# ChainBreak/denoising_diffusion_deep_fake

Measured on AMD Instinct MI355X. Metric: training images/sec (256x256 U-Net, bs=16/GPU), higher is better.
Workload: dtype f32; 1 GPU; d3f train_denoiser step: noise blend -> Unet(resnet34) fwd -> (MSE+1-SSIM)/2 -> bwd -> Adam, 256x256 synthetic face crops, bs=16/GPU, random-init weights, train-mode BatchNorm; image_size=256, batch_per_gpu=16, global_batch=16, parallelism=dp1, graph_step=False, adam_overlap_tail=False, adam_overlap_tail_steps=0, ranks_seen=1, csrc_digest=87bcf01c09701563

## Files before the change

denoising_diffusion_deep_fake_amd/csrc/conv_wgrad_patch.hip:

```cpp
#include "common.h"

#include <cstdlib>

namespace d3f {

constexpr int PT_TH = 8;

template <int MT> struct PAcc;
template <> struct PAcc<32> { using T = f32x16; static constexpr int N = 16; };
template <> struct PAcc<16> { using T = f32x4; static constexpr int N = 4; };

template <int MT> __device__ __forceinline__ void pmma(typename PAcc<MT>::T& c, float a, float b);
template <> __device__ __forceinline__ void pmma<32>(f32x16& c, float a, float b) {
  c = __builtin_amdgcn_mfma_f32_32x32x2f32(a, b, c, 0, 0, 0);
}
template <> __device__ __forceinline__ void pmma<16>(f32x4& c, float a, float b) {
  c = __builtin_amdgcn_mfma_f32_16x16x4f32(a, b, c, 0, 0, 0);
}

template <typename T> __device__ __forceinline__ void patch_store_f32(float* dst, const uint4& v);
template <> __device__ __forceinline__ void patch_store_f32<float>(float* dst, const uint4& v) {
  *reinterpret_cast<uint4*>(dst) = v;
}
template <> __device__ __forceinline__ void patch_store_f32<bf16_t>(float* dst, const uint4& v) {
  *reinterpret_cast<uint4*>(dst) = make_uint4(v.x << 16, v.x & 0xffff0000u, v.y << 16, v.y & 0xffff0000u);
  *reinterpret_cast<uint4*>(dst + 4) = make_uint4(v.z << 16, v.z & 0xffff0000u, v.w << 16, v.w & 0xffff0000u);
}

template <typename T, int MT, int CI_T, int KS, int S, int TW, int CR = CI_T>
__global__ __launch_bounds__(256) void conv_wgrad_patch_kernel(const WgradParams pin) {
  const WgradParams p = wgrad_params_of_net(pin, (int)blockIdx.z);
  constexpr int VE = Elem<T>::VE;
  constexpr int CO_T = MT;
  constexpr bool HALFV = CI_T < VE;
  static_assert(!HALFV || (CI_T == 4 && VE == 8), "half vectors: 4 of 8 bf16 channels");
  constexpr int PH = (PT_TH - 1) * S + KS, PW = (TW - 1) * S + KS;
  constexpr int KSTEP = (MT == 32) ? 2 : 4;
  static_assert(CR == CI_T || (CR < CI_T && CI_T < MT), "fewer columns than staged channels: small-channel path only");
  constexpr int NCOL = KS * KS * CR;
  constexpr int NNT = (NCOL + MT - 1) / MT;
  constexpr int LXS = (CI_T >= 32) ? (MT == 16 ? CI_T + 16 : CI_T + 4) : CI_T;
  constexpr int LYS = (MT == 32) ? CO_T + 4 : CO_T;
  constexpr int XF = PH * PW * LXS, YF = PT_TH * TW * LYS;
  constexpr int RED = 4 * MT * MT;
  constexpr int LDS_F = (XF + YF > RED) ? XF + YF : RED;
  __shared__ __attribute__((aligned(16))) float lds[LDS_F];
  float* Xs = lds;
  float* Ys = lds + XF;

  const int tid = threadIdx.x, lane = tid & 63, wave = tid >> 6;
  const int lc = lane & (MT - 1);
  const int lg = lane / MT;
  const int Cin = p.slab_cin;
  const int ci_slices = HALFV ? 1 : Cin / CI_T;
  const int slice = blockIdx.y;
  const int cil0 = (slice % ci_slices) * CI_T;
  const int ci0 = p.ci_base + cil0, co0 = (slice / ci_slices) * CO_T;
  const bool from0 = ci0 < p.C0;
  const int Cs = from0 ? p.C0 : p.C1;
  const int sh = from0 ? p.shift0 : 0;
  const int Hs = from0 ? p.H0s : p.Hv;
  const int Ws = from0 ? p.W0s : p.Wv;
  const int cl0 = from0 ? ci0 : ci0 - p.C0;
  const __amdgpu_buffer_rsrc_t rdy = make_rsrc(p.dy, p.dy_bytes);
  const __amdgpu_buffer_rsrc_t rx = from0 ? make_rsrc(p.src0, p.src0_bytes) : make_rsrc(p.src1, p.src1_bytes);

  int loff[(CI_T >= MT) ? 1 : NNT];
  if (CI_T < MT) {
#pragma unroll
    for (int j = 0; j < NNT; ++j) {
      const int n = j * MT + lc;
      int tap = n / CR;
      const int c = n - tap * CR;
      if (tap >= KS * KS) tap = KS * KS - 1;
      const int kh = tap / KS, kw = tap - kh * KS;
      loff[(CI_T >= MT) ? 0 : j] = (kh * PW + kw) * LXS + c;
    }
  }

  typename PAcc<MT>::T acc[NNT];
#pragma unroll
  for (int j = 0; j < NNT; ++j)
#pragma unroll
    for (int r = 0; r < PAcc<MT>::N; ++r) acc[j][r] = 0.f;

  const int tiles_x = (p.Wo + TW - 1) / TW, tiles_y = (p.Ho + PT_TH - 1) / PT_TH;
  const int ntiles = p.B * tiles_y * tiles_x;
  constexpr int VX = HALFV ? 1 : CI_T / VE, VY = CO_T / VE;

  constexpr int NVX = (PH * PW * VX + 255) / 256, NVY = (PT_TH * TW * VY + 255) / 256;
  uint4 rxv[NVX], ryv[NVY];
  auto issue_loads = [&](int t) {
    const int b = t / (tiles_y * tiles_x);
    const int tr = t - b * tiles_y * tiles_x;
    const int oy0 = (tr / tiles_x) * PT_TH, ox0 = (tr % tiles_x) * TW;
#pragma unroll
    for (int i = 0; i < NVX; ++i) {
      const int v = tid + i * 256;
      const int pix = v / VX, cv = v - pix * VX;
      const int py = pix / PW, px = pix - py * PW;
      const int iy = oy0 * S - p.pad + py, ix = ox0 * S - p.pad + px;
      const bool ok = v < PH * PW * VX && (unsigned)iy < (unsigned)p.Hv && (unsigned)ix < (unsigned)p.Wv;
      const int gp = (b * Hs + (iy >> sh)) * Ws + (ix >> sh);
      rxv[i] = buf_load16(rx, ok ? (unsigned)(gp * Cs + cl0 + cv * VE) * (unsigned)sizeof(T) : BUF_OOB);
    }
#pragma unroll
    for (int i = 0; i < NVY; ++i) {
      const int v = tid + i * 256;
      const int pix = v / VY, cv = v - pix * VY;
      const int y = pix / TW, x = pix - y * TW;
      const int oy = oy0 + y, ox = ox0 + x;
      const int co = co0 + cv * VE;
      const bool ok = v < PT_TH * TW * VY && oy < p.Ho && ox < p.Wo && co < p.Cout;
      ryv[i] = buf_load16(rdy, ok ? (unsigned)(((b * p.Ho + oy) * p.Wo + ox) * p.Cout + co) * (unsigned)sizeof(T) : BUF_OOB);
    }
  };
  auto store_tile = [&]() {
#pragma unroll
    for (int i = 0; i < NVX; ++i) {
      const int v = tid + i * 256;
      const int pix = v / VX, cv = v - pix * VX;
      if (v < PH * PW * VX) {
        if constexpr (HALFV)
          *reinterpret_cast<uint4*>(&Xs[pix * LXS]) =
              make_uint4(rxv[i].x << 16, rxv[i].x & 0xffff0000u, rxv[i].y << 16, rxv[i].y & 0xffff0000u);
        else
          patch_store_f32<T>(&Xs[pix * LXS + cv * VE], rxv[i]);
      }
    }
#pragma unroll
    for (int i = 0; i < NVY; ++i) {
      const int v = tid + i * 256;
      const int pix = v / VY, cv = v - pix * VY;
      if (v < PT_TH * TW * VY) patch_store_f32<T>(&Ys[pix * LYS + cv * VE], ryv[i]);
    }
  };

  if ((int)blockIdx.x < ntiles) issue_loads(blockIdx.x);
  for (int t = blockIdx.x; t < ntiles; t += gridDim.x) {
    __syncthreads();
    store_tile();
    __syncthreads();
    if (t + (int)gridDim.x < ntiles) issue_loads(t + gridDim.x);
#pragma unroll
    for (int yy = 0; yy < PT_TH / 4; ++yy) {
      const int y = wave * (PT_TH / 4) + yy;
      const float* __restrict__ yrow = Ys + (y * TW + lg) * LYS + lc;
      const float* __restrict__ xrow = Xs + ((y * S) * PW + lg * S) * LXS + ((CI_T >= MT) ? lc : 0);
#pragma unroll
      for (int xs = 0; xs < TW / KSTEP; ++xs) {
        const float a = yrow[xs * KSTEP * LYS];
        const float* __restrict__ xb = xrow + xs * KSTEP * S * LXS;
#pragma unroll
        for (int j = 0; j < NNT; ++j) {
          float bv;
          if (CI_T >= MT) {
            constexpr int per_tap = CI_T / MT;
            const int tap = j / per_tap, cb = (j % per_tap) * MT;
            const int kh = tap / KS, kw = tap % KS;
            bv = xb[(kh * PW + kw) * LXS + cb];
          } else {
            bv = xb[loff[(CI_T >= MT) ? 0 : j]];
          }
          pmma<MT>(acc[j], a, bv);
        }
      }
    }
  }

  const int taps = KS * KS;
  float* __restrict__ slab = p.partial + (long)blockIdx.x * p.Cout * taps * Cin;
  float* red = lds;
#pragma unroll
  for (int j = 0; j < NNT; ++j) {
    __syncthreads();
#pragma unroll
    for (int r = 0; r < PAcc<MT>::N; ++r) {
      const int co_l = (MT == 32) ? ((r & 3) + 8 * (r >> 2) + 4 * lg) : (4 * lg + r);
      red[(wave * MT + co_l) * MT + lc] = acc[j][r];
    }
    __syncthreads();
    for (int e = tid; e < MT * MT; e += 256) {
      const float s = (red[e] + red[MT * MT + e]) + (red[2 * MT * MT + e] + red[3 * MT * MT + e]);
      const int co = co0 + e / MT;
      const int n = j * MT + (e % MT);
      const int tap = n / CR, ci = cil0 + (n - tap * CR);
      if (co < p.Cout && tap < taps) {
        slab[((long)co * taps + tap) * Cin + ci] = s;
        if constexpr (HALFV && CR == CI_T) slab[((long)co * taps + tap) * Cin + ci + CI_T] = 0.f;
      }
    }
  }
  if constexpr (CR < CI_T) {
    const int npad = Cin - CR;
    for (int e = tid; e < MT * taps * npad; e += 256) {
      const int c = CR + e % npad, q = e / npad, tap = q % taps, co = co0 + q / taps;
      if (co < p.Cout) slab[((long)co * taps + tap) * Cin + c] = 0.f;
    }
  }
}

template <typename T, int MT, int CI_T, int TW>
__global__ __launch_bounds__(256) void conv_wgrad_patch_cls_kernel(const WgradParams pin) {
  const WgradParams p = wgrad_params_of_net(pin, (int)blockIdx.z);
  constexpr int VE = Elem<T>::VE;
  constexpr int CO_T = MT;
  constexpr int RH = PT_TH / 2;
  static_assert(RH == 4, "one tile row of the parity per wave");
  constexpr int PHL = PT_TH / 2 + 2, PWL = TW / 2 + 2;
  constexpr int KSTEP = (MT == 32) ? 2 : 4;
  constexpr int NCT = CI_T / MT;
  constexpr int NNT = 8 * NCT;
  static_assert(CI_T % MT == 0, "whole column tiles per folded tap");
  constexpr int LXS = (MT == 16 ? CI_T + 16 : CI_T + 4);
  constexpr int LYS = (MT == 32) ? CO_T + 4 : CO_T;
  constexpr int XF = PHL * PWL * LXS, YF = RH * TW * LYS;
  constexpr int RED = 4 * MT * MT;
  constexpr int LDS_F = (XF + YF > RED) ? XF + YF : RED;
  __shared__ __attribute__((aligned(16))) float lds[LDS_F];
  float* Xs = lds;
  float* Ys = lds + XF;

  const int tid = threadIdx.x, lane = tid & 63, wave = tid >> 6;
  const int lc = lane & (MT - 1);
  const int lg = lane / MT;
  const int Cin = p.slab_cin;
  const int ci_slices = Cin / CI_T;
  int slice = blockIdx.y;
  const int py = slice & 1;
  slice >>= 1;
  const int ci0 = (slice % ci_slices) * CI_T, co0 = (slice / ci_slices) * CO_T;
  const __amdgpu_buffer_rsrc_t rdy = make_rsrc(p.dy, p.dy_bytes);
  const __amdgpu_buffer_rsrc_t rx = make_rsrc(p.src0, p.src0_bytes);

  typename PAcc<MT>::T acc[NNT];
#pragma unroll
  for (int j = 0; j < NNT; ++j)
#pragma unroll
    for (int r = 0; r < PAcc<MT>::N; ++r) acc[j][r] = 0.f;

  const int tiles_x = (p.Wo + TW - 1) / TW, tiles_y = (p.Ho + PT_TH - 1) / PT_TH;
  const int ntiles = p.B * tiles_y * tiles_x;
  constexpr int VX = CI_T / VE, VY = CO_T / VE;
  constexpr int NVX = (PHL * PWL * VX + 255) / 256, NVY = (RH * TW * VY + 255) / 256;
  uint4 rxv[NVX], ryv[NVY];
  auto issue_loads = [&](int t) {
    const int b = t / (tiles_y * tiles_x);
    const int tr = t - b * tiles_y * tiles_x;
    const int oy0 = (tr / tiles_x) * PT_TH, ox0 = (tr % tiles_x) * TW;
    const int ly0 = oy0 / 2 - 1, lx0 = ox0 / 2 - 1;
#pragma unroll
    for (int i = 0; i < NVX; ++i) {
      const int v = tid + i * 256;
      const int pix = v / VX, cv = v - pix * VX;
      const int yy = pix / PWL, xx = pix - yy * PWL;
      const int iy = ly0 + yy, ix = lx0 + xx;
      const bool ok = v < PHL * PWL * VX && (unsigned)iy < (unsigned)p.H0s && (unsigned)ix < (unsigned)p.W0s;
      const int gp = (b * p.H0s + iy) * p.W0s + ix;
      rxv[i] = buf_load16(rx, ok ? (unsigned)(gp * p.C0 + ci0 + cv * VE) * (unsigned)sizeof(T) : BUF_OOB);
    }
#pragma unroll
    for (int i = 0; i < NVY; ++i) {
      const int v = tid + i * 256;
      const int pix = v / VY, cv = v - pix * VY;
      const int r = pix / TW, x = pix - r * TW;
      const int oy = oy0 + 2 * r + py, ox = ox0 + x;
      const int co = co0 + cv * VE;
      const bool ok = v < RH * TW * VY && oy < p.Ho && ox < p.Wo && co < p.Cout;
      ryv[i] = buf_load16(rdy, ok ? (unsigned)(((b * p.Ho + oy) * p.Wo + ox) * p.Cout + co) * (unsigned)sizeof(T) : BUF_OOB);
    }
  };
  auto store_tile = [&]() {
#pragma unroll
    for (int i = 0; i < NVX; ++i) {
      const int v = tid + i * 256;
      const int pix = v / VX, cv = v - pix * VX;
      if (v < PHL * PWL * VX) patch_store_f32<T>(&Xs[pix * LXS + cv * VE], rxv[i]);
    }
#pragma unroll
    for (int i = 0; i < NVY; ++i) {
      const int v = tid + i * 256;
      const int pix = v / VY, cv = v - pix * VY;
      if (v < RH * TW * VY) patch_store_f32<T>(&Ys[pix * LYS + cv * VE], ryv[i]);
    }
  };

  if ((int)blockIdx.x < ntiles) issue_loads(blockIdx.x);
  for (int t = blockIdx.x; t < ntiles; t += gridDim.x) {
    __syncthreads();
    store_tile();
    __syncthreads();
    if (t + (int)gridDim.x < ntiles) issue_loads(t + gridDim.x);
    const float* __restrict__ yrow = Ys + (wave * TW) * LYS + lc;
#pragma unroll
    for (int px = 0; px < 2; ++px) {
#pragma unroll
      for (int xs = 0; xs < (TW / 2) / KSTEP; ++xs) {
        const int il = lg + xs * KSTEP;
        const float a = yrow[(2 * il + px) * LYS];
#pragma unroll
        for (int fa = 0; fa < 2; ++fa)
#pragma unroll
          for (int fb = 0; fb < 2; ++fb) {
            const float* __restrict__ xb = Xs + ((wave + fa + py) * PWL + il + fb + px) * LXS + lc;
#pragma unroll
            for (int jc = 0; jc < NCT; ++jc) pmma<MT>(acc[((px * 2 + fa) * 2 + fb) * NCT + jc], a, xb[jc * MT]);
          }
      }
    }
  }

  float* __restrict__ slab = p.partial + (long)blockIdx.x * p.Cout * 16 * Cin;
  float* red = lds;
#pragma unroll
  for (int j = 0; j < NNT; ++j) {
    __syncthreads();
#pragma unroll
    for (int r = 0; r < PAcc<MT>::N; ++r) {
      const int co_l = (MT == 32) ? ((r & 3) + 8 * (r >> 2) + 4 * lg) : (4 * lg + r);
      red[(wave * MT + co_l) * MT + lc] = acc[j][r];
    }
    __syncthreads();
    const int f8 = j / NCT, jc = j - f8 * NCT;
    const int tap = py * 8 + f8;
    for (int e = tid; e < MT * MT; e += 256) {
      const float s = (red[e] + red[MT * MT + e]) + (red[2 * MT * MT + e] + red[3 * MT * MT + e]);
      const int co = co0 + e / MT;
      const int ci = ci0 + jc * MT + (e % MT);
      if (co < p.Cout) slab[((long)co * 16 + tap) * Cin + ci] = s;
    }
  }
}


constexpr int PB_TW = 16;
__global__ __launch_bounds__(256) void conv_wgrad_patch_bf16_kernel(const WgradParams pin) {
  const WgradParams p = wgrad_params_of_net(pin, (int)blockIdx.z);
  typedef short v4s __attribute__((ext_vector_type(4)));
  constexpr int TW = PB_TW, KS = 3, PH = PT_TH + 2, PW = TW + 2;
  constexpr int XB = PH * PW * 64, YB = PT_TH * TW * 64;
  constexpr int RED = 4 * 32 * 32;
  constexpr int LDS_B = (XB + YB > RED * 4) ? XB + YB : RED * 4;
  __shared__ __attribute__((aligned(16))) unsigned char ldsb[LDS_B];
  unsigned char* Xs = ldsb;
  unsigned char* Ys = ldsb + XB;

  const int tid = threadIdx.x, lane = tid & 63, wave = tid >> 6;
  const int Cin = p.slab_cin;
  const int ci_slices = (Cin + 31) / 32;
  const int slice = blockIdx.y;
  const int cil0 = (slice % ci_slices) * 32;
  const int ci0 = p.ci_base + cil0, co0 = (slice / ci_slices) * 32;
  const bool from0 = ci0 < p.C0;
  const int Cs = from0 ? p.C0 : p.C1;
  const int sh = from0 ? p.shift0 : 0;
  const int Hs = from0 ? p.H0s : p.Hv;
  const int Ws = from0 ? p.W0s : p.Wv;
  const int cl0 = from0 ? ci0 : ci0 - p.C0;
  const int xreal = min(32, Cs - cl0), yreal = min(32, p.Cout - co0);
  const __amdgpu_buffer_rsrc_t rdy = make_rsrc(p.dy, p.dy_bytes);
  const __amdgpu_buffer_rsrc_t rx = from0 ? make_rsrc(p.src0, p.src0_bytes) : make_rsrc(p.src1, p.src1_bytes);

  f32x16 acc[KS * KS];
#pragma unroll
  for (int j = 0; j < KS * KS; ++j)
#pragma unroll
    for (int r = 0; r < 16; ++r) acc[j][r] = 0.f;

  const int tiles_x = (p.Wo + TW - 1) / TW, tiles_y = (p.Ho + PT_TH - 1) / PT_TH;
  const int ntiles = p.B * tiles_y * tiles_x;
  constexpr int NVX = (PH * PW * 4 + 255) / 256, NVY = (PT_TH * TW * 4 + 255) / 256;
  uint4 rxv[NVX], ryv[NVY];
  auto issue_loads = [&](int t) {
    const int b = t / (tiles_y * tiles_x);
    const int tr = t - b * tiles_y * tiles_x;
    const int oy0 = (tr / tiles_x) * PT_TH, ox0 = (tr % tiles_x) * TW;
#pragma unroll
    for (int i = 0; i < NVX; ++i) {
      const int v = tid + i * 256;
      const int pix = v >> 2, cv = v & 3;
      const int py = pix / PW, px = pix - py * PW;
      const int iy = oy0 - p.pad + py, ix = ox0 - p.pad + px;
      const bool ok = v < PH * PW * 4 && cv * 8 < xreal && (unsigned)iy < (unsigned)p.Hv && (unsigned)ix < (unsigned)p.Wv;
      const int gp = (b * Hs + (iy >> sh)) * Ws + (ix >> sh);
      rxv[i] = buf_load16(rx, ok ? (unsigned)(gp * Cs + cl0 + cv * 8) * 2u : BUF_OOB);
    }
#pragma unroll
    for (int i = 0; i < NVY; ++i) {
      const int v = tid + i * 256;
      const int pix = v >> 2, cv = v & 3;
      const int y = pix / TW, x = pix - y * TW;
      const int oy = oy0 + y, ox = ox0 + x;
      const bool ok = v < PT_TH * TW * 4 && cv * 8 < yreal && oy < p.Ho && ox < p.Wo;
      ryv[i] = buf_load16(rdy, ok ? (unsigned)(((b * p.Ho + oy) * p.Wo + ox) * p.Cout + co0 + cv * 8) * 2u : BUF_OOB);
    }
  };
  auto store_tile = [&]() {
#pragma unroll
    for (int i = 0; i < NVX; ++i) {
      const int v = tid + i * 256;
      if (v < PH * PW * 4) *reinterpret_cast<uint4*>(Xs + v * 16) = rxv[i];
    }
#pragma unroll
    for (int i = 0; i < NVY; ++i) {
      const int v = tid + i * 256;
      if (v < PT_TH * TW * 4) *reinterpret_cast<uint4*>(Ys + v * 16) = ryv[i];
    }
  };
  const int lg = lane >> 4, q = (lane & 15) >> 2, pq = lane & 3;
  const int rd_lane = ((lg >> 1) * 8 + q) * 64 + ((lg & 1) * 16 + 4 * pq) * 2;
  auto frag = [&](const unsigned char* base) {
    union { uint4 u; v4s h[2]; } f;
#pragma unroll
    for (int h = 0; h < 2; ++h)
      f.h[h] = __builtin_amdgcn_ds_read_tr16_b64_v4i16((__attribute__((address_space(3))) v4s*)(base + rd_lane + h * 4 * 64));
    return f.u;
  };

  if ((int)blockIdx.x < ntiles) issue_loads(blockIdx.x);
  for (int t = blockIdx.x; t < ntiles; t += gridDim.x) {
    __syncthreads();
    store_tile();
    __syncthreads();
    if (t + (int)gridDim.x < ntiles) issue_loads(t + gridDim.x);
#pragma unroll
    for (int yy = 0; yy < PT_TH / 4; ++yy) {
      const int y = wave * (PT_TH / 4) + yy;
      const uint4 a = frag(Ys + (y * TW) * 64);
#pragma unroll
      for (int tap = 0; tap < KS * KS; ++tap) {
        const int kh = tap / KS, kw = tap - kh * KS;
        const uint4 b = frag(Xs + ((y + kh) * PW + kw) * 64);
        acc[tap] = __builtin_amdgcn_mfma_f32_32x32x16_bf16(*reinterpret_cast<const bf16x8*>(&a),
                                                           *reinterpret_cast<const bf16x8*>(&b), acc[tap], 0, 0, 0);
      }
    }
  }

  const int taps = KS * KS;
  float* __restrict__ slab = p.partial + (long)blockIdx.x * p.Cout * taps * Cin;
  float* red = reinterpret_cast<float*>(ldsb);
  const int lc = lane & 31, lh = lane >> 5;
#pragma unroll
  for (int j = 0; j < KS * KS; ++j) {
    __syncthreads();
#pragma unroll
    for (int r = 0; r < 16; ++r) red[(wave * 32 + (r & 3) + 8 * (r >> 2) + 4 * lh) * 32 + lc] = acc[j][r];
    __syncthreads();
    for (int e = tid; e < 32 * 32; e += 256) {
      const float sum = (red[e] + red[1024 + e]) + (red[2048 + e] + red[3072 + e]);
      const int co = co0 + (e >> 5), cil = e & 31;
      if (co < p.Cout && cil < xreal) slab[((long)co * taps + j) * Cin + cil0 + cil] = sum;
    }
  }
}

int wgrad_patch_variant(const WgradParams& p, int dtype) {
  const int cin = p.C0 + p.C1;
  if (p.KH != p.KW) return 0;
  constexpr int maxco = 128;
  constexpr int maxci = 384;
  if (dtype == D3F_BF16 && p.KH == 3 && p.stride == 1 && p.pad == 1 && p.Cout <= maxco && (cin == 16 || (cin % 32 == 0 && cin <= maxci)) &&
      (p.C1 == 0 || p.C0 % 32 == 0) && (p.C0 % 8) == 0 && (p.C1 % 8) == 0 && (p.Cout % 8) == 0)
    return 7;
  if (p.KH == 3 && p.stride == 1 && p.pad == 1) {
    if (p.Cout <= 16 && cin % 32 == 0 && cin <= 64 && (p.C1 == 0 || p.C0 % 32 == 0)) return 1;
    if (p.Cout <= 16 && cin == 16) return 2;
    if (p.Cout == 32 && cin % 32 == 0 && cin <= 128 && (p.C1 == 0 || p.C0 % 32 == 0)) return 3;
  }
  if (dtype == D3F_F32 && p.KH == 7 && p.stride == 2 && p.pad == 3 && cin == 4 && p.C1 == 0 &&
      p.Cout % 32 == 0 && p.Cout <= 64)
    return 4;
  if (dtype == D3F_BF16 && p.KH == 7 && p.stride == 2 && p.pad == 3 && cin == 8 && p.C1 == 0 &&
      p.Cout % 32 == 0 && p.Cout <= 64)
    return (p.cin_real > 0 && p.cin_real <= 4) ? 6 : 5;
  return 0;
}

int wgrad_patch_tiles(const WgradParams& p) { return p.B * cdiv(p.Ho, PT_TH) * cdiv(p.Wo, 16); }

void wgrad_patch_grid(const WgradParams& p, int variant, int* gx, int* gy) {
  const int cin = p.part == WG_WHOLE ? p.C0 + p.C1 : p.part == WG_CLASS ? p.C0 : p.C1;
  const int ci_t = variant == 1 ? 32 : variant == 2 ? 16 : (variant == 3 || variant == 7) ? 32 : (variant == 5 || variant == 6) ? 8 : 4;
  const int co_t = (variant == 3 || variant == 4 || variant == 5 || variant == 6 || variant == 7) ? 32 : 16;
  const int slices = cdiv(cin, ci_t) * cdiv(p.Cout, co_t) * (p.part == WG_CLASS ? 2 : 1);
  const int tiles = wgrad_patch_tiles(p);
  constexpr int g7 = 256;
  static const int gall = prof_knob("D3F_WGRAD_PATCH_WGS") ? atoi(prof_knob("D3F_WGRAD_PATCH_WGS")) : 512;
  int g = (variant == 7 ? g7 : gall) / plan_nets_for(p.plan_nets, 32) / slices;
  if (g > tiles) g = tiles;
  if (g < 1) g = 1;
  *gx = g;
  *gy = slices;
}

template <typename T> static int patch_launch_t(const WgradParams& p, int variant, dim3 grid, hipStream_t stream) {
  const dim3 block(256);
  switch (variant) {
    case 1: hipLaunchKernelGGL((conv_wgrad_patch_kernel<T, 16, 32, 3, 1, 16>), grid, block, 0, stream, p); break;
    case 2: hipLaunchKernelGGL((conv_wgrad_patch_kernel<T, 16, 16, 3, 1, 16>), grid, block, 0, stream, p); break;
    case 3: hipLaunchKernelGGL((conv_wgrad_patch_kernel<T, 32, 32, 3, 1, 16>), grid, block, 0, stream, p); break;
    default: return set_error(-1, "wgrad patch: bad variant %d", variant);
  }
  return 0;
}

int wgrad_patch_launch(const WgradParams& p, int variant, int dtype, hipStream_t stream) {
  int gx, gy;
  wgrad_patch_grid(p, variant, &gx, &gy);
  D3F_CHECK(p.splits == gx, "wgrad patch: params were not planned (splits %d vs %d)", p.splits, gx);
  const dim3 grid((unsigned)gx, (unsigned)gy, (unsigned)nets_of(p.nets)), block(256);
  if (p.cls) {
    D3F_CHECK((variant == 1 || variant == 3) && p.slab_cin == p.C0 && (p.C0 % 32) == 0 && (p.Ho % 2) == 0 && (p.Wo % 2) == 0,
              "wgrad patch: class form needs variant 1 or 3 and whole 32-channel slices of source 0");
    if (dtype == D3F_F32) {
      if (variant == 1) hipLaunchKernelGGL((conv_wgrad_patch_cls_kernel<float, 16, 32, 16>), grid, block, 0, stream, p);
      else hipLaunchKernelGGL((conv_wgrad_patch_cls_kernel<float, 32, 32, 16>), grid, block, 0, stream, p);
    } else {
      if (variant == 1) hipLaunchKernelGGL((conv_wgrad_patch_cls_kernel<bf16_t, 16, 32, 16>), grid, block, 0, stream, p);
      else hipLaunchKernelGGL((conv_wgrad_patch_cls_kernel<bf16_t, 32, 32, 16>), grid, block, 0, stream, p);
    }
    D3F_HIP(hipGetLastError());
    return 0;
  }
  if (variant == 7) {
    D3F_CHECK(dtype == D3F_BF16 && p.part == WG_WHOLE, "wgrad patch: variant 7 is the native bf16 kernel of whole layers");
    hipLaunchKernelGGL(conv_wgrad_patch_bf16_kernel, grid, block, 0, stream, p);
  } else if (variant == 4) {
    D3F_CHECK(dtype == D3F_F32, "wgrad patch: stem variant 4 is the f32 one");
    if (p.cin_real == 3) hipLaunchKernelGGL((conv_wgrad_patch_kernel<float, 32, 4, 7, 2, 16, 3>), grid, block, 0, stream, p);
    else hipLaunchKernelGGL((conv_wgrad_patch_kernel<float, 32, 4, 7, 2, 16>), grid, block, 0, stream, p);
  } else if (variant == 5) {
    D3F_CHECK(dtype == D3F_BF16, "wgrad patch: stem variant 5 is the bf16 one");
    hipLaunchKernelGGL((conv_wgrad_patch_kernel<bf16_t, 32, 8, 7, 2, 16>), grid, block, 0, stream, p);
  } else if (variant == 6) {
    D3F_CHECK(dtype == D3F_BF16, "wgrad patch: stem variant 6 is a bf16 one");
    if (p.cin_real == 3) hipLaunchKernelGGL((conv_wgrad_patch_kernel<bf16_t, 32, 4, 7, 2, 16, 3>), grid, block, 0, stream, p);
    else hipLaunchKernelGGL((conv_wgrad_patch_kernel<bf16_t, 32, 4, 7, 2, 16>), grid, block, 0, stream, p);
  } else if (dtype == D3F_F32) {
    if (int rc = patch_launch_t<float>(p, variant, grid, stream)) return rc;
  } else {
    if (int rc = patch_launch_t<bf16_t>(p, variant, grid, stream)) return rc;
  }
  D3F_HIP(hipGetLastError());
  return 0;
}

}
```

denoising_diffusion_deep_fake_amd/csrc/engine.hip:

```cpp
#include "engine.h"
#include <vector>

#include "head_act.h"

#include <cstdio>
#include <cstdlib>
#include <cstring>

namespace d3f {

constexpr int CS_PP = 16;
__global__ __launch_bounds__(256) void channel_sum_partial_kernel(const float* __restrict__ x, int C, long HW,
                                                                  float* __restrict__ partial, int nb, long net_in,
                                                                  long net_ws) {
  __shared__ float red[256];
  const int seg = blockIdx.x, c = blockIdx.y, b = (int)blockIdx.z % nb;
  if ((int)blockIdx.z >= nb) {
    net_shift(x, net_in); net_shift(partial, net_ws);
  }
  const float* __restrict__ plane = x + ((long)b * C + c) * HW;
  const long per = (HW + CS_PP - 1) / CS_PP, lo = (long)seg * per, hi = lo + per < HW ? lo + per : HW;
  float s = 0.f;
  if ((HW & 3) == 0 && (per & 3) == 0) {
    for (long i = lo + 4 * threadIdx.x; i < hi; i += 4 * 256) {
// ... 644 lines not shown
  frame_.color = mode;
  return 0;
}

int UnetEngine::set_frame_temporal(float strength, int threshold) {
  D3F_CHECK(strength >= 0.f && strength < 1.f, "frame temporal filter: strength %g outside [0, 1) (0 is off)",
            (double)strength);
  D3F_CHECK(threshold >= 1 && threshold <= 255, "frame temporal filter: threshold %d outside 1..255", threshold);
  if (strength == 0.f) strength = 0.f;
  if (memcmp(&strength, &frame_.strength, sizeof(float)) == 0 && threshold == frame_.threshold) return 0;
  if (strength != 0.f) {
    const size_t px = (size_t)H * W;
    D3F_HIP(frame_.state_fake.ensure(px * 3 * sizeof(float)));
    D3F_HIP(frame_.state_real.ensure(px * 3));
    D3F_HIP(frame_.state_coef.ensure(6 * sizeof(float)));
    D3F_HIP(frame_.state_sum.ensure(3 * sizeof(uint64_t)));
    D3F_HIP(frame_.valid.ensure(2 * sizeof(int)));
  }
  drop_frame_graphs();
  frame_.strength = strength;
  frame_.threshold = threshold;
  frame_.reset_pending = true;
  return 0;
}

int UnetEngine::frame_temporal_reset(hipStream_t s) const {
  frame_.reset_pending = false;
  int* valid = frame_.valid.p;
  if (valid == nullptr) return 0;
  if (int rc = temporal_flag_set_launch(valid, 0, s)) return rc;
  return temporal_flag_set_launch(valid + 1, 0, s);
}

void UnetEngine::GraphSlot::destroy() {
  if (exec) (void)hipGraphExecDestroy(exec);
  exec = nullptr;
}

void UnetEngine::drop_frame_graphs() const {
  g_frames_.destroy();
  g_frames_full_.destroy();
}

void UnetEngine::drop_graphs() const {
  g_predict_.destroy();
  g_eval_.destroy();
  drop_frame_graphs();
  if (g_step_) {
    (void)hipGraphExecDestroy(g_step_);
    g_step_ = nullptr;
  }
}

struct Scale255 {
  float mean[3], stdv[3];
  Scale255(const float m[3], const float sd[3]) {
    for (int c = 0; c < 3; ++c) {
      mean[c] = m[c] * 255.0f;
      stdv[c] = sd[c] * 255.0f;
    }
  }
};

int UnetEngine::predict_u8(const float* params_, float* bnstats, const uint8_t* bgr_in, uint8_t* bgr_out,
                           const float mean[3], const float stdv[3], void* ws_, int use_graph,
                           hipStream_t s) const {
  D3F_CHECK(in_channels == 3 && classes == 3, "predict_u8: 3-channel frames only (in %d, out %d)", in_channels, classes);
  char* ws = reinterpret_cast<char*>(ws_);
  const Scale255 k(mean, stdv);
  if (!use_graph) return predict_u8_launches(params_, bnstats, bgr_in, bgr_out, k.mean, k.stdv, ws, s);
  const GraphKey key = {{params_, bnstats, bgr_in, bgr_out, ws_},
                        {k.mean[0], k.mean[1], k.mean[2], k.stdv[0], k.stdv[1], k.stdv[2]}, {}};
  return graph_replay(g_predict_, key, s, [&](hipStream_t gs) {
    return predict_u8_launches(params_, bnstats, bgr_in, bgr_out, k.mean, k.stdv, ws, gs);
  });
}

int UnetEngine::predict_frames(const FrameCall& c, const float* params_, float* bnstats, const float mean[3],
                               const float stdv[3], void* ws_, int use_graph, hipStream_t s) const {
  const bool full = c.full_out != nullptr;
  const char* who = full ? "predict_frames_full_u8" : "predict_frames_u8";
  D3F_CHECK(in_channels == 3 && classes == 3, "%s: 3-channel frames only (in %d, out %d)", who, in_channels, classes);
  char* ws = reinterpret_cast<char*>(ws_);
  const Scale255 k(mean, stdv);
  const FrameOptions& o = frame_;
  const bool aa = o.resample == FRAME_RESAMPLE_CUBIC_AA;
  const bool color = full && o.color == FRAME_COLOR_MEANSTD;
  const bool temporal = o.strength != 0.f;
  uint8_t* const pair = c.pair_out;
  uint8_t* const fake = pair + pair_fake_off();
  const long stride = pair_stride();
  const int32_t* const boxes = c.boxes;
  D3F_CHECK(!(use_graph && boxes),
            "%s with a box per frame cannot be replayed from a graph: a captured launch bakes its kernel arguments in, the "
            "boxes among them, and a graph keyed on their values would be re-captured on every call; pass use_graph = 0",
            who);
  if (int rc = boxes ? (aa ? crop_resize_cubic_aa_boxes_check : crop_resize_cubic_boxes_check)(B, c.src_h, c.src_w, boxes, H,
                                                                                              W, stride)
                     : (aa ? crop_resize_cubic_aa_check : crop_resize_cubic_check)(B, c.src_h, c.src_w, c.x1, c.y1, c.cw,
                                                                                  c.ch, H, W, stride))
    return rc;
  if (full) {
    int rc;
    if (boxes)
      rc = color ? paste_resize_cubic_color_boxes_check(fake, c.raw_in, c.full_out, o.color_coef.p, B, H, W, stride, c.src_h,
                                                        c.src_w, boxes, c.feather)
                 : paste_resize_cubic_boxes_check(fake, c.raw_in, c.full_out, B, H, W, stride, c.src_h, c.src_w, boxes,
                                                  c.feather);
    else
      rc = color ? paste_resize_cubic_color_check(fake, c.raw_in, c.full_out, o.color_coef.p, B, H, W, stride, c.src_h,
                                                  c.src_w, c.x1, c.y1, c.cw, c.ch, c.feather)
                 : paste_resize_cubic_check(fake, c.raw_in, c.full_out, B, H, W, stride, c.src_h, c.src_w, c.x1, c.y1, c.cw,
                                            c.ch, c.feather);
    if (rc) return rc;
    D3F_CHECK(!(use_graph && c.full_out == c.raw_in),
              "predict_frames_full_u8: full_out == raw_in (in place) cannot be replayed from a graph: pass use_graph = 0");
  }
  if (temporal) {
    if (int rc = temporal_filter_check(pair, fake, B, H, W, stride, stride, o.state_fake.p, o.state_real.p, o.valid.p,
                                       o.strength, o.threshold))
      return rc;
    if (o.reset_pending)
      if (int rc = frame_temporal_reset(s)) return rc;
  }
  auto launches = [&](hipStream_t ls) {
    if (int rc = boxes ? (aa ? crop_resize_cubic_aa_boxes_u8_nhwc_launch : crop_resize_cubic_boxes_u8_nhwc_launch)(
                             dtype, c.raw_in, B, c.src_h, c.src_w, boxes, pair, H, W, stride, ws + tensors[t_x].off,
                             tensors[t_x].C, k.mean, k.stdv, ls)
                       : (aa ? crop_resize_cubic_aa_u8_nhwc_launch : crop_resize_cubic_u8_nhwc_launch)(
                             dtype, c.raw_in, B, c.src_h, c.src_w, c.x1, c.y1, c.cw, c.ch, pair, H, W, stride,
                             ws + tensors[t_x].off, tensors[t_x].C, k.mean, k.stdv, ls))
      return rc;
    float* head_out = reinterpret_cast<float*>(ws + head_nchw_off);
    if (int rc = forward_body(params_, bnstats, head_out, ws, 0, ls, nullptr, false)) return rc;
    head_z_live_ = false;
    if (int rc = head_to_u8bgr(ws, fake, stride, k.mean, k.stdv, ls)) return rc;
    if (temporal)
      if (int rc = temporal_filter_u8_launch(pair, fake, B, H, W, stride, stride, o.state_fake.p, o.state_real.p, o.valid.p,
                                             o.strength, o.threshold, ls))
        return rc;
    if (!full) return 0;
    if (!color)
      return boxes ? paste_resize_cubic_boxes_u8_launch(fake, B, H, W, stride, c.raw_in, c.src_h, c.src_w, boxes, c.feather,
                                                        c.full_out, ls)
                   : paste_resize_cubic_u8_launch(fake, B, H, W, stride, c.raw_in, c.src_h, c.src_w, c.x1, c.y1, c.cw, c.ch,
                                                  c.feather, c.full_out, ls);
    int parts = 0;
    if (int rc = channel_sums_pair_slabs_launch(pair, pair_fake_off(), B, H, W, stride, o.color_slabs.p, &parts, ls)) return rc;
    const uint64_t* to = o.color_slabs.p;
    const uint64_t* from = to + (size_t)B * parts * 6;
    if (int rc = color_match_coef_launch(from, to, parts, B, (long)H * W, o.color_coef.p, ls)) return rc;
    if (temporal)
      if (int rc = color_coef_smooth_launch(o.color_coef.p, to, parts, B, (long)H * W, o.strength, o.state_coef.p,
                                            o.state_sum.p, o.valid.p + 1, ls))
        return rc;
    if (boxes)
      return paste_resize_cubic_color_boxes_u8_launch(fake, B, H, W, stride, c.raw_in, c.src_h, c.src_w, boxes, c.feather,
                                                      o.color_coef.p, c.full_out, ls);
    return paste_resize_cubic_color_u8_launch(fake, B, H, W, stride, c.raw_in, c.src_h, c.src_w, c.x1, c.y1, c.cw, c.ch,
                                              c.feather, o.color_coef.p, c.full_out, ls);
  };
  if (!use_graph) return launches(s);
  int strength_bits;
  memcpy(&strength_bits, &o.strength, sizeof(strength_bits));
  const GraphKey key = {{params_, bnstats, c.raw_in, pair, ws_, c.full_out},
                        {k.mean[0], k.mean[1], k.mean[2], k.stdv[0], k.stdv[1], k.stdv[2]},
                        {c.src_h, c.src_w, c.x1, c.y1, c.cw, c.ch, full ? c.feather : 0, full ? o.color : 0, strength_bits,
                         temporal ? o.threshold : 0}};
  return graph_replay(full ? g_frames_full_ : g_frames_, key, s, launches);
}

int UnetEngine::forward_graph(const float* params_, float* bnstats, const float* x, float* out, void* ws_,
                              hipStream_t s) const {
  const GraphKey key = {{params_, bnstats, x, out, ws_}, {}, {}};
  return graph_replay(g_eval_, key, s, [&](hipStream_t gs) { return forward(params_, bnstats, x, out, ws_, 0, gs); });
}

int UnetEngine::train_step_launches(const StepArgs& a, void* ws_, hipStream_t s) const {
  const long per_image = (long)in_channels * H * W;
  if (int rc = pack_weights(a.params, ws_, s)) return rc;
  if (int rc = noise_blend_launch(a.image, a.noise, a.y_uniform, a.lam, a.noisy, nullptr, B, per_image, s)) return rc;
  if (int rc = forward(a.params, a.bnstats, a.noisy, a.pred, ws_, 1, s)) return rc;
  if (int rc = mse_ssim_loss_launch(a.pred, a.image, a.lo, a.hi, a.loss_out, a.gpred, a.loss_ws, B, H, W, s)) return rc;
  if (int rc = backward(a.params, a.gpred, a.grads, ws_, 0, num_segments, s, 1)) return rc;
  return adam_step_dev_launch(a.params, a.grads, a.exp_avg, a.exp_avg_sq, param_floats, a.adam_coef, s);
}

int UnetEngine::train_step(const StepArgs& a, void* ws_, int use_graph, hipStream_t s) const {
  D3F_CHECK(in_channels == 3 && classes == 3, "train_step: the (MSE + 1 - SSIM) / 2 objective is defined on 3-channel images");
  if (!use_graph) return train_step_launches(a, ws_, s);
  if (int rc = wait_for_packed_weights(s)) return rc;
  if (int rc = ensure_streams()) return rc;
  if (gstream_ == nullptr) {
    D3F_HIP(hipStreamCreateWithFlags(&gstream_, hipStreamNonBlocking));
    D3F_HIP(hipEventCreateWithFlags(&ev_gin_, hipEventDisableTiming));
    D3F_HIP(hipEventCreateWithFlags(&ev_gout_, hipEventDisableTiming));
  }
  const bool same = g_step_ != nullptr && g_step_ws_ == ws_ && memcmp(&a, &g_step_key_, sizeof(StepArgs)) == 0;
  if (!same) {
    if (g_step_) {
      (void)hipGraphExecDestroy(g_step_);
      g_step_ = nullptr;
    }
    hipGraph_t graph = nullptr;
    D3F_HIP(hipStreamBeginCapture(gstream_, hipStreamCaptureModeThreadLocal));
    const int rc = train_step_launches(a, ws_, gstream_);
    const hipError_t e = hipStreamEndCapture(gstream_, &graph);
    pack_pending_ = pack_mid_pending_ = false;
    side_dirty_ = false;
    if (rc != 0) {
      if (graph) (void)hipGraphDestroy(graph);
      return rc;
    }
    D3F_HIP(e);
    const hipError_t ei = hipGraphInstantiate(&g_step_, graph, nullptr, nullptr, 0);
    (void)hipGraphDestroy(graph);
    D3F_HIP(ei);
    g_step_key_ = a;
    g_step_ws_ = ws_;
  }
  D3F_HIP(hipGraphLaunch(g_step_, s));
  return 0;
}

int UnetEngine::wait_for_packed_weights(hipStream_t s) const {
  if (pack_mid_pending_) {
    D3F_HIP(hipStreamWaitEvent(s, ev_pack_mid_, 0));
    pack_mid_pending_ = false;
  }
  if (pack_pending_) {
    D3F_HIP(hipStreamWaitEvent(s, ev_pack_done_, 0));
    pack_pending_ = false;
  }
  return 0;
}

template <typename F>
int UnetEngine::graph_replay(GraphSlot& slot, const GraphKey& key, hipStream_t s, F&& launches) const {
  if (int rc = wait_for_packed_weights(s)) return rc;
  if (gstream_ == nullptr) {
    D3F_HIP(hipStreamCreateWithFlags(&gstream_, hipStreamNonBlocking));
    D3F_HIP(hipEventCreateWithFlags(&ev_gin_, hipEventDisableTiming));
    D3F_HIP(hipEventCreateWithFlags(&ev_gout_, hipEventDisableTiming));
  }
  static_assert(sizeof(GraphKey) == 6 * sizeof(void*) + 6 * sizeof(float) + 10 * sizeof(int), "GraphKey is compared bytewise");
  const bool same = slot.exec != nullptr && memcmp(&key, &slot.key, sizeof(GraphKey)) == 0;
  if (!same) {
    slot.destroy();
    hipGraph_t graph = nullptr;
    D3F_HIP(hipStreamBeginCapture(gstream_, hipStreamCaptureModeThreadLocal));
    const int rc = launches(gstream_);
    const hipError_t e = hipStreamEndCapture(gstream_, &graph);
    if (rc != 0) {
      if (graph) (void)hipGraphDestroy(graph);
      return rc;
    }
    D3F_HIP(e);
    const hipError_t ei = hipGraphInstantiate(&slot.exec, graph, nullptr, nullptr, 0);
    (void)hipGraphDestroy(graph);
    D3F_HIP(ei);
    slot.key = key;
  }
  D3F_HIP(hipEventRecord(ev_gin_, s));
  D3F_HIP(hipStreamWaitEvent(gstream_, ev_gin_, 0));
  D3F_HIP(hipGraphLaunch(slot.exec, gstream_));
  D3F_HIP(hipEventRecord(ev_gout_, gstream_));
  D3F_HIP(hipStreamWaitEvent(s, ev_gout_, 0));
  return 0;
}

UnetEngine::~UnetEngine() {
  drop_graphs();
  if (ev_gin_) (void)hipEventDestroy(ev_gin_);
  if (ev_gout_) (void)hipEventDestroy(ev_gout_);
  if (gstream_) (void)hipStreamDestroy(gstream_);
  for (hipEvent_t e : ev_dy_)
    if (e) (void)hipEventDestroy(e);
  if (ev_join_) (void)hipEventDestroy(ev_join_);
  if (ev_seg_) (void)hipEventDestroy(ev_seg_);
  if (ev_pack_in_) (void)hipEventDestroy(ev_pack_in_);
  if (ev_pack_done_) (void)hipEventDestroy(ev_pack_done_);
  if (ev_pack_mid_) (void)hipEventDestroy(ev_pack_mid_);
}

static bool serial_backward() {
  static const bool serial = getenv("D3F_SERIAL_BACKWARD") != nullptr;
  return serial;
}

hipStream_t UnetEngine::side_stream() const {
  if (serial_backward() || ensure_streams() != 0) return nullptr;
  return side_;
}

int UnetEngine::backward_join(hipStream_t s) const {
  if (side_ != nullptr && side_dirty_) {
    D3F_HIP(hipEventRecord(ev_join_, side_));
    D3F_HIP(hipStreamWaitEvent(s, ev_join_, 0));
    side_dirty_ = false;
  }
  return 0;
}

int UnetEngine::backward(const float* params_, const float* dout, float* grads, void* ws_,
                         int seg_begin, int seg_end, hipStream_t s, int join, const NetIO* io) const {
  char* ws = reinterpret_cast<char*>(ws_);
  D3F_CHECK(nets == 1 || (io != nullptr && bn_sync() == nullptr), "unet: the pair engine needs the second network's "
            "offsets and runs with per-GPU BatchNorm statistics");
  NetSplit split{};
  const NetSplit* ns = make_split(io, io ? io->dout : 0, &split) ? &split : nullptr;
  const bool head_act = head_act_ != HEAD_ACT_IDENTITY;
  const float* head_dz = head_act ? reinterpret_cast<const float*>(ws + head_nchw_off) : dout;
  NetSplit split_dz = split;
  split_dz.in = split_dz.ws;
  const NetSplit* ns_dz = (ns && head_act) ? &split_dz : ns;
  auto T = [&](int tid) { return ws + tensors[tid].off; };
  auto G = [&](int gid) { return gid == -2 ? ws + dz_off : ws + gtensors[gid].off; };
  auto coef = [&](const Unit& u) { return reinterpret_cast<float*>(ws + u.coef_off); };
  const bool serial = serial_backward();
#ifdef D3F_PROFILING
  static const char* abl = getenv("D3F_ABLATE_BACKWARD");
  const bool skip_w = abl && strchr(abl, 'w'), skip_d = abl && strchr(abl, 'd'), skip_b = abl && strchr(abl, 'b');
  const bool skip_r = abl && strchr(abl, 'r');
#else
  constexpr bool skip_w = false, skip_d = false, skip_b = false, skip_r = false;
#endif
  if (!serial)
    if (int rc = ensure_streams()) return rc;
  hipStream_t ws_stream = serial ? s : side_;
  size_t next_event = 0;
  bool side_used = false;
  constexpr int defer = 3;
  std::vector<int> pending;
  int pending_segment = -1;
  bool head_bias_pending = false;
  auto flush_pending = [&]() -> int {
    if (pending.empty()) return 0;
    if (!serial) {
      if (next_event == ev_dy_.size()) {
        hipEvent_t e = nullptr;
        D3F_HIP(hipEventCreateWithFlags(&e, hipEventDisableTiming));
        ev_dy_.push_back(e);
      }
      D3F_HIP(hipEventRecord(ev_dy_[next_event], s));
      D3F_HIP(hipStreamWaitEvent(side_, ev_dy_[next_event], 0));
      ++next_event;
      side_used = true;
    }
    if (head_bias_pending) {
      const Unit& uh = units[head];
      if (int rc = channel_sum_nchw_launch(head_dz, B, uh.Cout, (long)uh.Ho * uh.Wo, reinterpret_cast<float*>(ws + bsum_off),
                                           grads + uh.bias_off, ws_stream, ns_dz))
        return rc;
      head_bias_pending = false;
    }
    for (int ui : pending) {
      const Unit& u = units[ui];
      WgradReduceBatch red;
      if (int rc = wgrad_layer_launch_deferred(u.wl, ws + u.dy_off, T(u.in0), u.in1 >= 0 ? T(u.in1) : nullptr,
                                               reinterpret_cast<float*>(ws + u.wslab_off), grads + u.w_off, u.Cout,
                                               u.CinReal, cdtype, red, ws_stream, ns))
        return rc;
      if (!skip_r)
        if (int rc = wgrad_reduce_batch_launch(red, ws_stream)) return rc;
    }
    pending.clear();
    return 0;
  };
  for (const BwdOp& op : bwd_ops) {
    if (op.segment < seg_begin || op.segment >= seg_end) continue;
    if (op.segment != pending_segment) {
      if (int rc = flush_pending()) return rc;
      pending_segment = op.segment;
    }
    if (op.kind == BW_SUM2X2) {
      if (int rc = sum2x2_launch(dtype, ws + dfull_off, G(op.dst0), B, op.Hl, op.Wl, op.C, s, ns)) return rc;
      continue;
    }
    if (op.kind == BW_POOL) {
      const TensorD& f1 = tensors[units[conv1].a];
      if (int rc = maxpool3x3s2_bwd_launch(dtype, G(op.dA), reinterpret_cast<uint8_t*>(ws + pool_idx_off),
                                           G(op.dst0), op.acc0 ? 1 : 0, B, f1.H, f1.W, f1.C, s, ns))
        return rc;
      continue;
    }
    const Unit& u = units[op.unit];
    char* dy = ws + u.dy_off;
    if (op.kind == BW_HEAD) {
      if (head_act) {
        D3F_CHECK(head_z_live_, "unet backward: the head's pre-activation output of the last training forward is gone (an "
                  "earlier backward pass turned it into dz, or an inference pass overwrote it): one backward pass per "
                  "training forward with an activated head");
        float* z = reinterpret_cast<float*>(ws + head_nchw_off);
        if (int rc = head_act_backward_launch(head_act_, dtype, z, dout, z, dy, B, u.Cout, u.Ho, u.Wo, u.CoutD, s, ns))
          return rc;
        head_z_live_ = false;
      } else {
        if (int rc = nchw_to_nhwc_launch(dtype, dout, dy, B, u.Cout, u.Ho, u.Wo, u.CoutD, s, ns)) return rc;
      }
      if (skip_w) {
        if (int rc = channel_sum_nchw_launch(head_dz, B, u.Cout, (long)u.Ho * u.Wo,
                                             reinterpret_cast<float*>(ws + bsum_off), grads + u.bias_off, s, ns_dz))
          return rc;
      } else {
        head_bias_pending = true;
      }
    } else if (!skip_b) {
      BnBufs n;
      n.stats = reinterpret_cast<float*>(ws + bnpart_off);
      n.gamma = params_ + u.g_off;
      n.coef = coef(u);
      n.y = T(u.y); n.a = u.a >= 0 ? T(u.a) : nullptr;
      n.dA = G(op.dA); n.dy = dy;
      n.dres = op.dres == -1 ? nullptr : G(op.dres); n.dres_acc = op.dres_acc ? 1 : 0;
      n.dgamma = grads + u.g_off; n.dbeta = grads + u.b_off;
      if (int rc = bn_layer_backward(u.norm, n, bn_sync(), s, ns)) return rc;
    }
    if (!skip_w) {
      pending.push_back(op.unit);
      if ((int)pending.size() >= defer)
        if (int rc = flush_pending()) return rc;
    }
    if (u.need_dgrad && !skip_d) {
      ConvDgradBufs d;
      d.dy = dy;
      d.w = ws + (u.upfold ? u.wd4_off : u.wd_off);
      d.w_skip = ws + u.wds_off;
      if (op.dst0_is_full_scratch) {
        d.dx0 = ws + dfull_off;
      } else {
        d.dx0 = G(op.dst0);
        d.acc0 = op.acc0 ? 1 : 0;
      }
      d.dx1 = op.dst1 >= 0 ? G(op.dst1) : nullptr;
      d.acc1 = op.acc1 ? 1 : 0;
      d.slabs = reinterpret_cast<float*>(ws + splitk_off);
      if (op.fuse_for_unit >= 0) {
        const Unit& uc = units[op.fuse_for_unit];
        d.bn_y = T(uc.y);
        d.bn_coef = bn_coef(coef(uc), uc.Cout, BN_MEAN);
        d.bn_partial = reinterpret_cast<float*>(ws + bnpart_off);
        d.bn_a = uc.norm.mask == BN_MASK_FROM_A ? T(uc.a) : nullptr;
      }
      if (int rc = conv_layer_dgrad(u, d, s, ns)) return rc;
    }
  }
  if (int rc = flush_pending()) return rc;
  if (!serial && side_used) side_dirty_ = true;
  if (!serial && !join) {
    D3F_HIP(hipEventRecord(ev_seg_, s));
    D3F_HIP(hipStreamWaitEvent(side_, ev_seg_, 0));
    side_dirty_ = true;
  } else if (!serial) {
    if (int rc = backward_join(s)) return rc;
  }
  return 0;
}

const TensorD* UnetEngine::find_export(const char* name) const {
  const std::string n(name);
  const size_t colon = n.rfind(':');
  if (colon == std::string::npos) return nullptr;
  const std::string un = n.substr(0, colon), kind = n.substr(colon + 1);
  if (kind != "y" && kind != "a" && kind != "da") return nullptr;
  for (const Unit& u : units) {
    if (u.conv_name != un) continue;
    const int tid = kind == "y" ? u.y : u.a;
    if (tid < 0) return nullptr;
    if (kind == "da") return grad_of[tid] >= 0 ? &gtensors[grad_of[tid]] : nullptr;
    return &tensors[tid];
  }
  return nullptr;
}

int UnetEngine::export_tensor(const char* name, const void* ws_, float* out_nchw, hipStream_t s) const {
  const TensorD* t = find_export(name);
  D3F_CHECK(t != nullptr, "export: no tensor named '%s' (expected '<conv name>:y|a|da')", name);
  return nhwc_to_nchw_launch(dtype, reinterpret_cast<const char*>(ws_) + t->off, out_nchw, B, t->C, t->H, t->W, t->C, s);
}

int UnetEngine::export_shape(const char* name, int32_t dims[3]) const {
  const TensorD* t = find_export(name);
  D3F_CHECK(t != nullptr, "export: no tensor named '%s' (expected '<conv name>:y|a|da')", name);
  dims[0] = t->C; dims[1] = t->H; dims[2] = t->W;
  return 0;
}

}
```

Baseline: 2078 images/sec.

## Double-buffer LDS reads in wgrad patch kernels and move tail wgrads to the caller stream

```diff
diff --git a/denoising_diffusion_deep_fake_amd/csrc/conv_wgrad_patch.hip b/denoising_diffusion_deep_fake_amd/csrc/conv_wgrad_patch.hip
--- a/denoising_diffusion_deep_fake_amd/csrc/conv_wgrad_patch.hip
+++ b/denoising_diffusion_deep_fake_amd/csrc/conv_wgrad_patch.hip
@@ -28,7 +28,8 @@
 }
 
 template <typename T, int MT, int CI_T, int KS, int S, int TW, int CR = CI_T>
-__global__ __launch_bounds__(256) void conv_wgrad_patch_kernel(const WgradParams pin) {
+__global__ __launch_bounds__(256) __attribute__((amdgpu_waves_per_eu((MT == 32 && CI_T == 32) ? 2 : 1)))
+void conv_wgrad_patch_kernel(const WgradParams pin) {
   const WgradParams p = wgrad_params_of_net(pin, (int)blockIdx.z);
   constexpr int VE = Elem<T>::VE;
   constexpr int CO_T = MT;
@@ -136,35 +137,49 @@
     }
   };
 
+  constexpr int NXS = TW / KSTEP, NK = (PT_TH / 4) * NXS;
+  static_assert(NK % 2 == 0, "two register sets: k-steps in pairs");
+  const float* __restrict__ yrow0 = Ys + (wave * (PT_TH / 4) * TW + lg) * LYS + lc;
+  const float* __restrict__ xrow0 = Xs + ((wave * (PT_TH / 4) * S) * PW + lg * S) * LXS + ((CI_T >= MT) ? lc : 0);
+  auto read_step = [&](int i, float& a, float (&bv)[NNT]) {
+    const int yy = i / NXS, xs = i - yy * NXS;
+    a = yrow0[(yy * TW + xs * KSTEP) * LYS];
+    const float* __restrict__ xb = xrow0 + ((yy * S) * PW + xs * KSTEP * S) * LXS;
+#pragma unroll
+    for (int j = 0; j < NNT; ++j) {
+      if (CI_T >= MT) {
+        constexpr int per_tap = CI_T / MT;
+        const int tap = j / per_tap, cb = (j % per_tap) * MT;
+        const int kh = tap / KS, kw = tap % KS;
+        bv[j] = xb[(kh * PW + kw) * LXS + cb];
+      } else {
+        bv[j] = xb[loff[(CI_T >= MT) ? 0 : j]];
+      }
+    }
+  };
+  auto mma_step = [&](float a, const float (&bv)[NNT]) {
+#pragma unroll
+    for (int j = 0; j < NNT; ++j) pmma<MT>(acc[j], a, bv[j]);
+  };
+
   if ((int)blockIdx.x < ntiles) issue_loads(blockIdx.x);
   for (int t = blockIdx.x; t < ntiles; t += gridDim.x) {
     __syncthreads();
     store_tile();
     __syncthreads();
     if (t + (int)gridDim.x < ntiles) issue_loads(t + gridDim.x);
-#pragma unroll
-    for (int yy = 0; yy < PT_TH / 4; ++yy) {
-      const int y = wave * (PT_TH / 4) + yy;
-      const float* __restrict__ yrow = Ys + (y * TW + lg) * LYS + lc;
-      const float* __restrict__ xrow = Xs + ((y * S) * PW + lg * S) * LXS + ((CI_T >= MT) ? lc : 0);
-#pragma unroll
-      for (int xs = 0; xs < TW / KSTEP; ++xs) {
-        const float a = yrow[xs * KSTEP * LYS];
-        const float* __restrict__ xb = xrow + xs * KSTEP * S * LXS;
-#pragma unroll
-        for (int j = 0; j < NNT; ++j) {
-          float bv;
-          if (CI_T >= MT) {
-            constexpr int per_tap = CI_T / MT;
-            const int tap = j / per_tap, cb = (j % per_tap) * MT;
-            const int kh = tap / KS, kw = tap % KS;
-            bv = xb[(kh * PW + kw) * LXS + cb];
-          } else {
-            bv = xb[loff[(CI_T >= MT) ? 0 : j]];
-          }
-          pmma<MT>(acc[j], a, bv);
-        }
+    float a0, a1, b0[NNT], b1[NNT];
+    read_step(0, a0, b0);
+#pragma unroll
+    for (int i = 0; i < NK; i += 2) {
+      read_step(i + 1, a1, b1);
+      __builtin_amdgcn_sched_barrier(0);
+      mma_step(a0, b0);
+      if (i + 2 < NK) {
+        read_step(i + 2, a0, b0);
+        __builtin_amdgcn_sched_barrier(0);
       }
+      mma_step(a1, b1);
     }
   }
 
@@ -285,28 +300,43 @@
     }
   };
 
+  constexpr int NXS = (TW / 2) / KSTEP, NK = 2 * NXS, NB = 4 * NCT;
+  static_assert(NK % 2 == 0, "two register sets: k-steps in pairs");
+  const float* __restrict__ yrow0 = Ys + (wave * TW + 2 * lg) * LYS + lc;
+  const float* __restrict__ xrow0 = Xs + ((wave + py) * PWL + lg) * LXS + lc;
+  auto read_step = [&](int i, float& a, float (&bv)[NB]) {
+    const int px = i / NXS, xs = i - px * NXS;
+    a = yrow0[(2 * xs * KSTEP + px) * LYS];
+#pragma unroll
+    for (int f = 0; f < 4; ++f)
+#pragma unroll
+      for (int jc = 0; jc < NCT; ++jc)
+        bv[f * NCT + jc] = xrow0[((f >> 1) * PWL + xs * KSTEP + (f & 1) + px) * LXS + jc * MT];
+  };
+  auto mma_step = [&](int i, float a, const float (&bv)[NB]) {
+    const int px = i / NXS;
+#pragma unroll
+    for (int f = 0; f < NB; ++f) pmma<MT>(acc[px * NB + f], a, bv[f]);
+  };
+
   if ((int)blockIdx.x < ntiles) issue_loads(blockIdx.x);
   for (int t = blockIdx.x; t < ntiles; t += gridDim.x) {
     __syncthreads();
     store_tile();
     __syncthreads();
     if (t + (int)gridDim.x < ntiles) issue_loads(t + gridDim.x);
-    const float* __restrict__ yrow = Ys + (wave * TW) * LYS + lc;
-#pragma unroll
-    for (int px = 0; px < 2; ++px) {
-#pragma unroll
-      for (int xs = 0; xs < (TW / 2) / KSTEP; ++xs) {
-        const int il = lg + xs * KSTEP;
-        const float a = yrow[(2 * il + px) * LYS];
-#pragma unroll
-        for (int fa = 0; fa < 2; ++fa)
-#pragma unroll
-          for (int fb = 0; fb < 2; ++fb) {
-            const float* __restrict__ xb = Xs + ((wave + fa + py) * PWL + il + fb + px) * LXS + lc;
-#pragma unroll
-            for (int jc = 0; jc < NCT; ++jc) pmma<MT>(acc[((px * 2 + fa) * 2 + fb) * NCT + jc], a, xb[jc * MT]);
-          }
+    float a0, a1, b0[NB], b1[NB];
+    read_step(0, a0, b0);
+#pragma unroll
+    for (int i = 0; i < NK; i += 2) {
+      read_step(i + 1, a1, b1);
+      __builtin_amdgcn_sched_barrier(0);
+      mma_step(i, a0, b0);
+      if (i + 2 < NK) {
+        read_step(i + 2, a0, b0);
+        __builtin_amdgcn_sched_barrier(0);
       }
+      mma_step(i + 1, a1, b1);
     }
   }
 
diff --git a/denoising_diffusion_deep_fake_amd/csrc/engine.hip b/denoising_diffusion_deep_fake_amd/csrc/engine.hip
--- a/denoising_diffusion_deep_fake_amd/csrc/engine.hip
+++ b/denoising_diffusion_deep_fake_amd/csrc/engine.hip
@@ -970,6 +970,10 @@
   return 0;
 }
 
+#ifndef D3F_TAIL_ON_CALLER
+#define D3F_TAIL_ON_CALLER 2
+#endif
+
 int UnetEngine::backward(const float* params_, const float* dout, float* grads, void* ws_,
                          int seg_begin, int seg_end, hipStream_t s, int join, const NetIO* io) const {
   char* ws = reinterpret_cast<char*>(ws_);
@@ -1002,7 +1006,25 @@
   std::vector<int> pending;
   int pending_segment = -1;
   bool head_bias_pending = false;
-  auto flush_pending = [&]() -> int {
+  static const int tail_on_caller = prof_knob("D3F_TAIL_ON_CALLER") ? atoi(prof_knob("D3F_TAIL_ON_CALLER")) : D3F_TAIL_ON_CALLER;
+  std::vector<int> held;
+  auto launch_wgrad = [&](int ui, hipStream_t st) -> int {
+    const Unit& u = units[ui];
+    WgradReduceBatch red;
+    if (int rc = wgrad_layer_launch_deferred(u.wl, ws + u.dy_off, T(u.in0), u.in1 >= 0 ? T(u.in1) : nullptr,
+                                             reinterpret_cast<float*>(ws + u.wslab_off), grads + u.w_off, u.Cout,
+                                             u.CinReal, cdtype, red, st, ns))
+      return rc;
+    if (!skip_r)
+      if (int rc = wgrad_reduce_batch_launch(red, st)) return rc;
+    return 0;
+  };
+  auto stem_is_next = [&](const BwdOp& op) {
+    for (const BwdOp* q = &op + 1; q < bwd_ops.data() + bwd_ops.size(); ++q)
+      if (q->kind == BW_UNIT || q->kind == BW_HEAD) return q->unit == conv1 && q->segment < seg_end;
+    return false;
+  };
+  auto flush_pending = [&](bool before_stem = false) -> int {
     if (pending.empty()) return 0;
     if (!serial) {
       if (next_event == ev_dy_.size()) {
@@ -1022,15 +1044,16 @@
         return rc;
       head_bias_pending = false;
     }
-    for (int ui : pending) {
-      const Unit& u = units[ui];
-      WgradReduceBatch red;
-      if (int rc = wgrad_layer_launch_deferred(u.wl, ws + u.dy_off, T(u.in0), u.in1 >= 0 ? T(u.in1) : nullptr,
-                                               reinterpret_cast<float*>(ws + u.wslab_off), grads + u.w_off, u.Cout,
-                                               u.CinReal, cdtype, red, ws_stream, ns))
-        return rc;
-      if (!skip_r)
-        if (int rc = wgrad_reduce_batch_launch(red, ws_stream)) return rc;
+    const size_t n = pending.size(), stem_here = pending.back() == conv1 ? 1 : 0;
+    size_t hold = 0;
+    if (!serial && (stem_here || before_stem) && (size_t)std::max(tail_on_caller, 0) > held.size())
+      hold = std::min((size_t)tail_on_caller - held.size(), n - stem_here);
+    for (size_t k = 0; k < n; ++k) {
+      if (k + stem_here + hold >= n && k + stem_here < n) {
+        held.push_back(pending[k]);
+        continue;
+      }
+      if (int rc = launch_wgrad(pending[k], ws_stream)) return rc;
     }
     pending.clear();
     return 0;
@@ -1038,7 +1061,7 @@
   for (const BwdOp& op : bwd_ops) {
     if (op.segment < seg_begin || op.segment >= seg_end) continue;
     if (op.segment != pending_segment) {
-      if (int rc = flush_pending()) return rc;
+      if (int rc = flush_pending(op.kind == BW_UNIT && op.unit == conv1)) return rc;
       pending_segment = op.segment;
     }
     if (op.kind == BW_SUM2X2) {
@@ -1087,7 +1110,7 @@
     if (!skip_w) {
       pending.push_back(op.unit);
       if ((int)pending.size() >= defer)
-        if (int rc = flush_pending()) return rc;
+        if (int rc = flush_pending(stem_is_next(op))) return rc;
     }
     if (u.need_dgrad && !skip_d) {
       ConvDgradBufs d;
@@ -1114,6 +1137,8 @@
     }
   }
   if (int rc = flush_pending()) return rc;
+  for (int ui : held)
+    if (int rc = launch_wgrad(ui, s)) return rc;
   if (!serial && side_used) side_dirty_ = true;
   if (!serial && !join) {
     D3F_HIP(hipEventRecord(ev_seg_, s));
```

Measured after the change: 2095 images/sec, median of 6. About the same (+0.8%).
